# WL-Amigo/waifu2x-converter-cpp

Measured on AMD Instinct MI355X. Metric: Mpixels/sec end-to-end scale2.0x 7-layer conv, higher is better.
Workload: dtype f32; 1 GPU; scale2x_1080p (BASELINE.json configs[1]): scale2.0x topology (1-32-32-64-64-128-128-1, synthetic seeded weights) on a 1920x1080 RGB frame -> Y plane nearest-2x -> 3840x2160 CNN plane, one frame per GPU per step

## Files before the change

### waifu2x-converter-cpp_amd/csrc/w2xc_wino4.hip

```cpp
#include "w2xc_kernels.h"
#include "w2xc_device.h"
#include "w2xc_launch.hpp"
#include "w2xc_layout.h"
#include "w2xc_wino4_math.h"

#include <type_traits>

#ifdef W4_TIMING
__device__ unsigned long long w4_stamps[2][8192];
#define W4_STAMP(idx) do { const int i_ = (idx); if (blockIdx.x == 0 && pt == 0 && lane == 0 && i_ < 8192) w4_stamps[bt][i_] = __builtin_amdgcn_s_memtime(); } while (0)
#else
#define W4_STAMP(idx) do { } while (0)
#endif
#ifndef W4P_T0
#define W4P_T0 3
#endif
#ifndef W4_PF
#define W4_PF 2
#endif
#ifndef W4_DMA4
#define W4_DMA4 1
#endif
#ifndef W4_ABL
#define W4_ABL 0
#endif

namespace {

typedef float f32x4u __attribute__((ext_vector_type(4), aligned(4)));

static constexpr __host__ __device__ int w4p_dd_of(int xi) { return 6 * ((xi % 18) / 3) + 3 * (xi / 18) + (xi % 18) % 3; }

}

static __device__ __forceinline__ void store16_sc1(float *p, f32x4 v) { asm volatile("global_store_dwordx4 %0, %1, off sc1\n\ts_nop 1" : : "v"(p), "v"(v) : "memory"); }
static __device__ __forceinline__ void store4_sc1(float *p, float v) { asm volatile("global_store_dword %0, %1, off sc1\n\ts_nop 1" : : "v"(p), "v"(v) : "memory"); }
static __device__ __forceinline__ void store16_sys(float *p, f32x4 v) { asm volatile("global_store_dwordx4 %0, %1, off sc0 sc1\n\ts_nop 1" : : "v"(p), "v"(v) : "memory"); }
static __device__ __forceinline__ void store4_sys(float *p, float v) { asm volatile("global_store_dword %0, %1, off sc0 sc1\n\ts_nop 1" : : "v"(p), "v"(v) : "memory"); }

template <int K, int N>
static __device__ __forceinline__ void load16_sc1_batch(f32x4 (&t)[N], unsigned voff, const char *const (&b)[N])
{
    if constexpr (K < N) {
        unsigned long long bc;
        asm volatile("s_mov_b64 %1, %3\n\tglobal_load_dwordx4 %0, %2, %1 sc1" : "=v"(t[K]), "=&s"(bc) : "v"(voff), "s"(b[K]) : "memory");
        load16_sc1_batch<K + 1, N>(t, voff, b);
    }
}
template <int K, int N>
static __device__ __forceinline__ void pin_batch(f32x4 (&t)[N])
{
    if constexpr (K < N) {
        asm volatile("" : "+v"(t[K]));
        pin_batch<K + 1, N>(t);
    }
}
template <int K, int N>
static __device__ __forceinline__ void sum_batch(f32x4 &v, const f32x4 (&t)[N])
{
    if constexpr (K < N) {
        v += t[K];
        sum_batch<K + 1, N>(v, t);
    }
}

struct W4ProgJob {
    const float *G; long long ts, gs, rs;
    float *out; long long out_rs;
    const float *bias;
    unsigned *flags; unsigned epoch;
    int g_h, g_w, g_off, wino_py, ngroups;
// ... 38 lines not shown
        pin_batch<0, 9 * NOB>(t1);
        auto finish = [&](bool on, const f32x4 (&t)[9 * NOB], int yy, int xx, bool whole) {
            if (!on) return;
            f32x4 v = {0.0f, 0.0f, 0.0f, 0.0f};
            sum_batch<0, 9 * NOB>(v, t);
            float *oq = outp + (long long)yy * out_rs + xx;
            if (whole) {
                f32x4 o;
#pragma unroll
                for (int e = 0; e < 4; e++) o[e] = leaky(v[e] + b);
                store16_sys(oq, o);
            } else {
                const int sh = xx - (g_w - 4);
                for (int e = 0; xx + e < g_w; e++) {
                    const int idx = sh + e;
                    const float ve = idx == 0 ? v[0] : idx == 1 ? v[1] : idx == 2 ? v[2] : v[3];
                    store4_sys(oq + e, leaky(ve + b));
                }
            }
        };
        finish(true, t0, yy0, xx0, whole0);
        finish(on1, t1, yy1, xx1, whole1);
    }
    unsigned *flags = reinterpret_cast<unsigned *>(uni64((unsigned long long)a.flags));
    if (flags) {
        asm volatile("s_waitcnt vmcnt(0)" ::: "memory");
        __builtin_amdgcn_s_barrier();
        asm volatile("" ::: "memory");
        if (tid == 0) __hip_atomic_store(flags + (jr * uni(a.ngroups) + jg), (unsigned)uni((int)a.epoch), __ATOMIC_RELAXED, __HIP_MEMORY_SCOPE_SYSTEM);
    }
}

template <int CIN, int COUT, bool OUT_PLANAR, bool IN_NHWC = false, bool FUSE7 = false, bool PROG = false>
__global__ void __launch_bounds__(512, 2) conv3x3_wino4(W2xcConvDesc d, int tiles_x, int nitems)
{
#define W4B_ONLY(...)
#define W4B_SEL(b_, s_) s_
#define W4B_OUT d.out
#include "w2xc_wino4_body.inc"
#undef W4B_OUT
#undef W4B_SEL
#undef W4B_ONLY
}

template <int CIN, int COUT, bool FUSE7>
__global__ void __launch_bounds__(512, 2) conv3x3_wino4_batch(W2xcConvDesc d, int tiles_x, int nitems, W2xcBatchDesc bd)
{
    constexpr bool OUT_PLANAR = true, IN_NHWC = false, PROG = false;
#define W4B_ONLY(...) __VA_ARGS__
#define W4B_SEL(b_, s_) b_
#define W4B_OUT (d.out + (long long)(item / bd.items) * bd.out_bs)
#include "w2xc_wino4_body.inc"
#undef W4B_OUT
#undef W4B_SEL
#undef W4B_ONLY
}

template <int CIN, int COUT, bool OUT_PLANAR, bool IN_NHWC>
__global__ void __launch_bounds__(512, 2) conv3x3_wino4_batch_l(W2xcConvDesc d, int tiles_x, int nitems, W2xcBatchDesc bd)
{
    constexpr bool FUSE7 = false, PROG = false;
#define W4B_ONLY(...) __VA_ARGS__
#define W4B_SEL(b_, s_) b_
#define W4B_OUT (d.out + (long long)(item / bd.items) * bd.out_bs)
#include "w2xc_wino4_body.inc"
#undef W4B_OUT
#undef W4B_SEL
#undef W4B_ONLY
}

#ifndef W2XC_WINO4_PART
#define W2XC_WINO4_PART -1
#endif
template <int CIN, int COUT, bool OUT_PLANAR, bool IN_NHWC = false, bool FUSE7 = false, bool PROG = false>
static hipError_t launch_wino4(const W2xcConvDesc &d, hipStream_t stream)
{
    const int tiles_x = (d.out_w + 31) / 32, tiles_y = (d.out_h + (d.wino_py & 3) + 15) / 16;
    const int nitems = tiles_x * tiles_y * (COUT / 64);
    constexpr size_t lds_bytes = 3 * (size_t)(11 * 1024) + 2 * (size_t)(36 * 1024) + 3 * (size_t)(18 * 1024) + COUT * 4 + (PROG ? 16 : 0);
    static_assert(lds_bytes <= 160 * 1024, "LDS budget");
    if constexpr (PROG) {
        if (!d.prog_cnt || !d.g_out || !d.g_bias || d.g_w < 4 || (long long)d.out_h * d.out_rs * 4 >= (1ll << 32)) return hipErrorInvalidValue;
        hipError_t em = hipMemsetAsync(d.prog_cnt, 0, w2xc_wino4_prog_counters(d.out_w, d.out_h, d.wino_py) * sizeof(unsigned), stream);
        if (em != hipSuccess) return em;
    }
    auto kern = conv3x3_wino4<CIN, COUT, OUT_PLANAR, IN_NHWC, FUSE7, PROG>;
    static W2xcLdsOptIn opt_in;
    const hipError_t e = opt_in(kern, lds_bytes);
    if (e != hipSuccess) return e;
    hipLaunchKernelGGL(kern, dim3(w2xc_persistent_grid(nitems)), dim3(512), lds_bytes, stream, d, tiles_x, nitems);
    return hipGetLastError();
}


hipError_t w2xc_launch_wino4_nhwc_out(const W2xcConvDesc &d, hipStream_t stream);
#if W2XC_WINO4_PART == 1 || W2XC_WINO4_PART == -1
hipError_t w2xc_launch_wino4_nhwc_out(const W2xcConvDesc &d, hipStream_t stream)
{
#ifdef W4P_SINGLE
    return hipErrorInvalidValue;
#else
    if (d.cin == 32 && d.in_ps == 32 && d.in_cs == 1)
        return d.cout == 64 ? launch_wino4<32, 64, false, true>(d, stream) : d.cout == 128 ? launch_wino4<32, 128, false, true>(d, stream) : hipErrorInvalidValue;
    switch (d.cin * 1000 + d.cout) {
    case 32064:  return launch_wino4<32, 64, false>(d, stream);
    case 32128:  return launch_wino4<32, 128, false>(d, stream);
    case 64064:  return launch_wino4<64, 64, false>(d, stream);
    case 64128:  return launch_wino4<64, 128, false>(d, stream);
    case 128064: return launch_wino4<128, 64, false>(d, stream);
    case 128128: return launch_wino4<128, 128, false>(d, stream);
    case 128256: return w2xc_launch_wino4_wide(d, stream);
    default: return hipErrorInvalidValue;
    }
#endif
}
#endif

#if W2XC_WINO4_PART == 7 || W2XC_WINO4_PART == -1
hipError_t w2xc_launch_wino4_wide(const W2xcConvDesc &d, hipStream_t stream)
{
    if (d.cin != 128 || d.cout != 256 || d.in_ps != 1 || d.out_ps != 256 || d.out_cs != 1 || d.out_terms == 9) return hipErrorInvalidValue;
    return launch_wino4<128, 256, false>(d, stream);
}
// ... 55 lines not shown
#ifndef W4P_SINGLE
    if (in_nhwc) return d.cout == 64 ? launch_wino4<32, 64, true, true>(d, stream) : d.cout == 128 ? launch_wino4<32, 128, true, true>(d, stream) : hipErrorInvalidValue;
#endif
#ifdef W4P_SINGLE
    return d.cin == 128 && d.cout == 128 ? launch_wino4<128, 128, true>(d, stream) : hipErrorInvalidValue;
#else
    switch (d.cin * 1000 + d.cout) {
    case 32064:  return launch_wino4<32, 64, true>(d, stream);
    case 32128:  return launch_wino4<32, 128, true>(d, stream);
    case 64064:  return launch_wino4<64, 64, true>(d, stream);
    case 64128:  return launch_wino4<64, 128, true>(d, stream);
    case 128064: return launch_wino4<128, 64, true>(d, stream);
    case 128128: return launch_wino4<128, 128, true>(d, stream);
    default: return hipErrorInvalidValue;
    }
#endif
}
#endif

template <int CIN, int COUT, bool FUSE7>
static hipError_t launch_wino4_batch(const W2xcConvDesc &d, W2xcBatchDesc b, hipStream_t stream)
{
    const int tiles_x = (d.out_w + 31) / 32, tiles_y = (d.out_h + (d.wino_py & 3) + 15) / 16;
    const long long items = (long long)tiles_x * tiles_y * (COUT / 64);
    if (items * b.batch >= (1ll << 31)) return hipErrorInvalidValue;
    b.items = (int)items;
    const int nitems = (int)(items * b.batch);
    constexpr size_t lds_bytes = 3 * (size_t)(11 * 1024) + 2 * (size_t)(36 * 1024) + 3 * (size_t)(18 * 1024) + COUT * 4;
    static_assert(lds_bytes <= 160 * 1024, "LDS budget");
    auto kern = conv3x3_wino4_batch<CIN, COUT, FUSE7>;
    static W2xcLdsOptIn opt_in;
    const hipError_t e = opt_in(kern, lds_bytes);
    if (e != hipSuccess) return e;
    hipLaunchKernelGGL(kern, dim3(w2xc_persistent_grid(nitems)), dim3(512), lds_bytes, stream, d, tiles_x, nitems, b);
    return hipGetLastError();
}

template <int CIN, int COUT, bool OUT_PLANAR, bool IN_NHWC>
static hipError_t launch_wino4_batch_l(const W2xcConvDesc &d, W2xcBatchDesc b, hipStream_t stream)
{
    const int tiles_x = (d.out_w + 31) / 32, tiles_y = (d.out_h + (d.wino_py & 3) + 15) / 16;
    const long long items = (long long)tiles_x * tiles_y * (COUT / 64);
    if (items * b.batch >= (1ll << 31)) return hipErrorInvalidValue;
    b.items = (int)items;
    const int nitems = (int)(items * b.batch);
    constexpr size_t lds_bytes = 3 * (size_t)(11 * 1024) + 2 * (size_t)(36 * 1024) + 3 * (size_t)(18 * 1024) + COUT * 4;
    static_assert(lds_bytes <= 160 * 1024, "LDS budget");
    auto kern = conv3x3_wino4_batch_l<CIN, COUT, OUT_PLANAR, IN_NHWC>;
    static W2xcLdsOptIn opt_in;
    const hipError_t e = opt_in(kern, lds_bytes);
    if (e != hipSuccess) return e;
    hipLaunchKernelGGL(kern, dim3(w2xc_persistent_grid(nitems)), dim3(512), lds_bytes, stream, d, tiles_x, nitems, b);
    return hipGetLastError();
}

hipError_t w2xc_launch_wino4_batch_nhwc_in(const W2xcConvDesc &d, W2xcBatchDesc b, hipStream_t stream);
#if W2XC_WINO4_PART == 5 || W2XC_WINO4_PART == -1
hipError_t w2xc_launch_wino4_batch_nhwc_in(const W2xcConvDesc &d, W2xcBatchDesc b, hipStream_t stream)
{
    if (d.out_ps == 1) return d.cout == 64 ? launch_wino4_batch_l<32, 64, true, true>(d, b, stream) : d.cout == 128 ? launch_wino4_batch_l<32, 128, true, true>(d, b, stream) : hipErrorInvalidValue;
    return d.cout == 64 ? launch_wino4_batch_l<32, 64, false, true>(d, b, stream) : d.cout == 128 ? launch_wino4_batch_l<32, 128, false, true>(d, b, stream) : hipErrorInvalidValue;
}
#endif

hipError_t w2xc_launch_wino4_batch_nhwc_out(const W2xcConvDesc &d, W2xcBatchDesc b, hipStream_t stream);
#if W2XC_WINO4_PART == 6 || W2XC_WINO4_PART == -1
hipError_t w2xc_launch_wino4_batch_nhwc_out(const W2xcConvDesc &d, W2xcBatchDesc b, hipStream_t stream)
{
    switch (d.cin * 1000 + d.cout) {
    case 64064:  return launch_wino4_batch_l<64, 64, false, false>(d, b, stream);
    case 64128:  return launch_wino4_batch_l<64, 128, false, false>(d, b, stream);
    case 128064: return launch_wino4_batch_l<128, 64, false, false>(d, b, stream);
    case 128128: return launch_wino4_batch_l<128, 128, false, false>(d, b, stream);
    default: return hipErrorInvalidValue;
    }
}
#endif

hipError_t w2xc_launch_wino4_batch_wide(const W2xcConvDesc &d, W2xcBatchDesc b, hipStream_t stream);
#if W2XC_WINO4_PART == 8 || W2XC_WINO4_PART == -1
hipError_t w2xc_launch_wino4_batch_wide(const W2xcConvDesc &d, W2xcBatchDesc b, hipStream_t stream)
{
    if (d.cin != 128 || d.cout != 256 || d.in_ps != 1 || d.out_ps != 256 || d.out_cs != 1 || d.out_terms == 9) return hipErrorInvalidValue;
    return launch_wino4_batch_l<128, 256, false, false>(d, b, stream);
}
// ... 57 lines not shown
```

### waifu2x-converter-cpp_amd/csrc/w2xc_wino4_body.inc

```
    static_assert(!PROG || FUSE7, "PROG finishes the fused last layer");
    constexpr int ROWS = 16;
    constexpr int NST = CIN / 4;
    constexpr int NOB = COUT / 64;
    constexpr int CHS = 168;
    constexpr int RAW_PIECES = 11;
    constexpr unsigned RAW_BYTES = RAW_PIECES * 1024;
    constexpr unsigned U_BASE = 3 * RAW_BYTES, U_BYTES = 36 * 1024;
    constexpr unsigned V_BASE = U_BASE + 2 * U_BYTES, V_BYTES = 18 * 1024;
    constexpr unsigned SPARE_BASE = V_BASE + 2 * V_BYTES;
    constexpr unsigned BIAS_BASE = SPARE_BASE + V_BYTES;
    static_assert(CIN % 16 == 0 && COUT % 64 == 0 && NST % 4 == 0 && NST >= 8, "planes");
    constexpr int STRIP = 16;
    constexpr int GW = 8;
    constexpr unsigned TRIG_BASE = BIAS_BASE + COUT * 4;
    const int tiles_y = W4B_SEL(bd.items, nitems) / (NOB * tiles_x);
    W4B_ONLY(const int img_tiles = bd.items / NOB;)
    const int pxcd = blockIdx.x & 7;
    auto band_lo = [&](int k, int r) { return (k * tiles_x + (r & 7)) >> 3; };
    auto tile_coords = [&](int pt_, int &ty_, int &tx_) {
        W4B_ONLY(pt_ = pt_ % img_tiles;)
        if constexpr (PROG) {
            const int p8 = pt_ / tiles_x;
            int rem = pt_ - p8 * tiles_x, j = 0, lo = band_lo(pxcd, 0), wd = band_lo(pxcd + 1, 0) - lo;
            while (rem >= wd && j < 7) {
                rem -= wd;
                j++;
                lo = band_lo(pxcd, j);
                wd = band_lo(pxcd + 1, j) - lo;
            }
            ty_ = 8 * p8 + j;
            tx_ = lo + rem;
            return;
        }
        const int per_strip = STRIP * tiles_y;
        int sidx = pt_ / per_strip;
        const int nfull = tiles_x / STRIP;
        if (sidx > nfull) sidx = nfull;
        const int wid = sidx < nfull ? STRIP : tiles_x - nfull * STRIP;
        const int q = pt_ - sidx * per_strip;
        ty_ = q / wid;
        tx_ = sidx * STRIP + (q - ty_ * wid);
    };
    extern __shared__ __attribute__((aligned(16))) float lds[];
    const unsigned lds0 = (unsigned)(size_t)(__attribute__((address_space(3))) float *)lds;
    char *ldsb = reinterpret_cast<char *>(lds);

    const int lane = threadIdx.x & 63;
    const int wave = __builtin_amdgcn_readfirstlane(threadIdx.x >> 6);
    const int pt = wave & 3, bt = wave >> 2;
    const unsigned b_voff = (unsigned)lane * 16u;
    auto lin = [&]() { unsigned v = b_voff; asm volatile("" : "+v"(v)); return v; };
    auto lane_o = [&]() { return (int)(lin() >> 4); };

    const int xcd = blockIdx.x & 7, per = gridDim.x >> 3;
    const int cq = nitems >> 3, cr = nitems & 7;
    int chunk_begin = xcd < cr ? xcd * (cq + 1) : cr * (cq + 1) + (xcd - cr) * cq;
    int chunk_end = chunk_begin + cq + (xcd < cr ? 1 : 0);
    if constexpr (PROG) {
        int nloc = (tiles_y >> 3) * tiles_x;
        for (int j = 0; j < (tiles_y & 7); j++) nloc += band_lo(xcd + 1, j) - band_lo(xcd, j);
        chunk_begin = 0;
        chunk_end = nloc * NOB;
    }
#ifndef W4_PAIR
#define W4_PAIR 0
#endif
    int item0 = chunk_begin + (blockIdx.x >> 3);
    int nmy = (chunk_end - item0 + per - 1) / per;
    if constexpr (W4_PAIR && NOB == 2 && !PROG) {
        const int ntile = nitems >> 1, tq = ntile >> 3, tr = ntile & 7;
        const int tb = xcd < tr ? xcd * (tq + 1) : tr * (tq + 1) + (xcd - tr) * tq, te = tb + tq + (xcd < tr ? 1 : 0);
        item0 = tb + (blockIdx.x >> 3);
        if (item0 >= te) return;
        nmy = 2 * ((te - item0 + per - 1) / per);
    } else if (item0 >= chunk_end) return;
    auto item_of = [&](int n) {
        const int nn = n < nmy ? n : nmy - 1;
        if constexpr (W4_PAIR && NOB == 2 && !PROG) return 2 * (item0 + (nn >> 1) * per) + (nn & 1);
        else return item0 + nn * per;
    };

    for (int c = threadIdx.x; c < COUT; c += 512) lds[BIAS_BASE / 4 + c] = d.bias[c];
    if constexpr (PROG) {
        if (threadIdx.x < 4) lds[TRIG_BASE / 4 + threadIdx.x] = 0.0f;
    }

    const long long cs4 = d.in_cs * 4, rs4 = d.in_rs * 4;
    constexpr int DW = W4_DMA4 ? 4 : 8;
    constexpr int RJ = (RAW_PIECES + DW - 1) / DW;
    constexpr int UQ = 36 / DW + (36 % DW ? 1 : 0);
    unsigned voff[RJ];
    const char *a_base;
    int xlim_r;
    auto tile_offsets = [&](int it) {
        int ty_, tx_;
        tile_coords(it / NOB, ty_, tx_);
        const int lane_t = lane_o();
        const int y0 = ty_ * ROWS - d.wino_py + d.off_y, x0 = tx_ * 32 + d.off_x;
        const int yb = clampi(y0, 0, d.in_h - 1);
        a_base = reinterpret_cast<const char *>(d.in) + (long long)yb * rs4;
        W4B_ONLY(a_base += (long long)(it / bd.items) * bd.in_bs * 4;)
        xlim_r = d.in_w - x0;
        if constexpr (IN_NHWC) {
            xlim_r = 64;
#pragma unroll
            for (int jj = 0; jj < RJ; jj++) {
                int ci = (jj * DW + wave) * 64 + lane_t;
                ci = ci < (ROWS + 2) * 36 ? ci : (ROWS + 2) * 36 - 1;
                const int R = ci / 36, slot = ci - R * 36;
                const int x = 4 * (slot % 9) + slot / 9;
                const int gy = clampi(y0 + R, 0, d.in_h - 1) - yb;
                const int gx = clampi(x0 + x, 0, d.in_w - 1);
                voff[jj] = (unsigned)((long long)gy * rs4 + (long long)gx * (CIN * 4));
            }
            return;
        }
        const int xq_last = (d.in_w - 1) & ~3;
#pragma unroll
        for (int jj = 0; jj < RJ; jj++) {
            const int ci = (jj * DW + wave) * 64 + lane_t;
            int kk = ci / CHS;
            kk = kk < 4 ? kk : 3;
            const int rem = ci - kk * CHS;
            int R = rem / 9;
            const int q = rem - R * 9;
            R = R < ROWS + 2 ? R : ROWS + 1;
            const int gy = clampi(y0 + R, 0, d.in_h - 1) - yb;
            int gx = x0 + 4 * q;
            gx = gx < xq_last ? gx : xq_last;
            voff[jj] = (unsigned)((long long)kk * cs4 + (long long)gy * rs4 + (long long)gx * 4);
        }
    };
    const unsigned wbase = (unsigned)__builtin_amdgcn_readfirstlane(lds0 + (unsigned)wave * 1024u);
    auto dma_raw = [&](auto JJ, unsigned roff, int slice) {
        constexpr int jj = decltype(JJ)::value;
        const char *sbase = a_base + (long long)slice * (IN_NHWC ? 16 : 4 * cs4);
        lds_dma16_si<jj * DW * 1024u>(sbase, voff[jj], wbase + roff);
    };
    const char *wpk_w = reinterpret_cast<const char *>(d.wpk) + (size_t)wave * 1024;
    auto dma_u = [&](int ob, int s_, auto SLOT, auto Q) {
        constexpr unsigned slot = decltype(SLOT)::value;
        constexpr int q = decltype(Q)::value;
        const char *sbase = wpk_w + ((size_t)(ob * NST + s_) * 36 + q * DW) * 1024;
        lds_dma16_si<U_BASE + slot * U_BYTES + q * DW * 1024u>(sbase, b_voff, wbase);
    };
#ifndef W4_DMA_BASES
#define W4_DMA_BASES 1
#endif
    constexpr bool DMAB = W4_DMA_BASES && W4_DMA4 && !(CIN == 32 && COUT == 128 && !OUT_PLANAR && !IN_NHWC && !FUSE7);
    auto dma_u_pair = [&](const char *u_pair, auto SLOT, auto Q) {
// ... 155 lines not shown

    auto run = [&](auto PH_) {
    constexpr int PH = decltype(PH_)::value;
    using C0 = std::integral_constant<int, 0>;
    using C1 = std::integral_constant<int, 1>;
    using U0 = std::integral_constant<unsigned, 0u>;
    lane_regs();
    const unsigned park_u = (bt * 3 + PH - 1) < 4 ? U_BASE + U_BYTES + (unsigned)(bt * 3 + PH - 1) * 9216u : SPARE_BASE + (unsigned)(bt * 3 + PH - 1 - 4) * 9216u;
    auto park = [&]() {
        char *pa = ldsb + (lin() + park_u);
        static_for<0, 9>([&](auto Q_) {
            constexpr int q = decltype(Q_)::value;
            *reinterpret_cast<f32x4 *>(pa + q * 1024) = f32x4{dd[4 * q], dd[4 * q + 1], dd[4 * q + 2], dd[4 * q + 3]};
        });
    };
    auto unpark = [&]() {
        const char *pa = ldsb + (lin() + park_u);
        static_for<0, 9>([&](auto Q_) {
            constexpr int q = decltype(Q_)::value;
            const f32x4 v = *reinterpret_cast<const f32x4 *>(pa + q * 1024);
            dd[4 * q] = v[0]; dd[4 * q + 1] = v[1]; dd[4 * q + 2] = v[2]; dd[4 * q + 3] = v[3];
        });
    };
    auto quarter = [&](auto Q_, const char *src, char *dst, int xlim) {
        constexpr int q = decltype(Q_)::value;
        if constexpr (q == 0) {
            static_for<0, 6>([&](auto I) { raw_read(src, I); });
            raw_mask(xlim);
        }
        if constexpr (q < 2) static_for<3 * q, 3 * q + 3>([&](auto I) { row_pass(I); });
        else static_for<3 * (q - 2), 3 * (q - 2) + 3>([&](auto J) { col_pass(J); });
        if constexpr (q == 3) static_for<0, 9>([&](auto Q) { v_write(dst, Q); });
    };
    tile_offsets(item_of(0));
    int xlim_cur = xlim_r;
    auto raw_all = [&](unsigned roff, int slice) {
        if (wave < DW) {
            static_for<0, RJ - 1>([&](auto JJ) { dma_raw(JJ, roff, slice); });
            if (wave < RAW_PIECES - (RJ - 1) * DW) dma_raw(std::integral_constant<int, RJ - 1>{}, roff, slice);
        }
    };
    for (int sl = 0; sl < 3; sl++) raw_all((unsigned)sl * RAW_BYTES, sl);
    if (wave < DW) {
        const int ob0 = item_of(0) % NOB;
        static_for<0, UQ - 1>([&](auto Q) { dma_u(ob0, 0, U0{}, Q); });
        if (wave < 36 - (UQ - 1) * DW) dma_u(ob0, 0, U0{}, std::integral_constant<int, UQ - 1>{});
    }
    W2XC_WAIT_VMCNT(0);
    __builtin_amdgcn_s_barrier();
    asm volatile("" ::: "memory");
    if constexpr (PH < 3) {
        const char *src = ldsb + PH * RAW_BYTES + tr_rd();
        static_for<0, 4 - PH>([&](auto Q) { quarter(Q, src, ldsb + tr_wr(), xlim_cur); });
    }
    asm volatile("s_waitcnt lgkmcnt(0)" ::: "memory");
    __builtin_amdgcn_s_barrier();
    asm volatile("" ::: "memory");
    for (int sl = 3; sl < 6; sl++) raw_all((unsigned)(sl - 3) * RAW_BYTES, sl);
    W2XC_WAIT_VMCNT(0);
    __builtin_amdgcn_s_barrier();
    asm volatile("" ::: "memory");
    if constexpr (PH == 3) quarter(C0{}, ldsb + tr_rd(), nullptr, xlim_cur);
    asm volatile("s_waitcnt lgkmcnt(0)" ::: "memory");
    __builtin_amdgcn_s_barrier();
    asm volatile("" ::: "memory");

    constexpr int PF = W4_PF;
// ... 4 lines not shown
        const char *va = va_of(slot);
        static_for<0, PF>([&](auto G) {
            constexpr int g = decltype(G)::value;
            const int b = PF == 2 ? g : (int)slot;
            a4[b] = *reinterpret_cast<const f32x4 *>(ua + g * 4096);
            b4[b] = *reinterpret_cast<const f32x4 *>(va + g * 2048);
        });
    };
    unsigned rd = RAW_BYTES, mid = 2 * RAW_BYTES, fr = 0;
    int stamp = 0;
    (void)stamp;
    W4_STAMP(stamp++);
    for (int n = 0; n < nmy; n++) {
        const int item = item_of(n), item_n = item_of(n + 1);
        f32x4 acc[36];

        auto stage = [&](auto J_, auto FIRST_, int s) {
            constexpr int J = decltype(J_)::value;
            constexpr bool FIRST = decltype(FIRST_)::value;
            constexpr int QT = (J - PH) & 3;
            constexpr unsigned par = J & 1, nxt = par ^ 1u;
            int u_ob = item % NOB, u_s = s + 1;
            if (s == NST - 1) { u_ob = item_n % NOB; u_s = 0; }
            const char *ua = ua_of(par);
            const char *va = va_of(par);
            const char *u_st = wpk_w + (size_t)(u_ob * NST + u_s) * 36864, *u_pair = u_st;
            if constexpr (DMAB) asm volatile("" : "+s"(u_st));
            const char *srcQ = nullptr;
            char *dstQ = nullptr;
            if constexpr (QT == 0) srcQ = ldsb + (rd + tr_rd());
            if constexpr (QT == 3) dstQ = ldsb + (tr_wr() + nxt * V_BYTES);
            const int xlimQ = s + 4 < NST ? xlim_cur : xlim_r;
            if constexpr (J == 2) {
                if (s == NST - 6) tile_offsets(item_n);
            }
            const int r_slice = s + 6 < NST ? s + 6 : s + 6 - NST;
            static_for<0, 36>([&](auto XI) {
                constexpr int xi = decltype(XI)::value;
                constexpr int g = xi >> 2;
                if constexpr (xi == 32) {
                    W4_STAMP(stamp++);
                    if constexpr ((W4_ABL & 32) != 0) W2XC_WAIT_VMCNT(0);
                    else if (wave < RAW_PIECES - (RJ - 1) * DW) wait_vmcnt_n(RJ);
                    else if (wave < DW) wait_vmcnt_n(RJ - 1);
                    asm volatile("s_waitcnt lgkmcnt(0)" ::: "memory");
                    W4_STAMP(stamp++);
                    __builtin_amdgcn_s_barrier();
                    asm volatile("" ::: "memory");
                    { const unsigned tr = rd; rd = mid; mid = fr; fr = tr; }
                    if (s != NST - 1) {
                        if constexpr (PF == 2) load_first(nxt);
                        else {
                            a4[nxt] = *reinterpret_cast<const f32x4 *>(ua_of(nxt));
                            b4[nxt] = *reinterpret_cast<const f32x4 *>(va_of(nxt));
                        }
                    }
                    W4_STAMP(stamp++);
                    __builtin_amdgcn_sched_barrier(0);
                }
                if constexpr ((xi & 3) == 0 && g + PF < 9 && !(W4_ABL & 128)) {
                    constexpr int b = PF == 2 ? (g + PF) % 3 : ((g + 1 + (int)par) & 1);
                    a4[b] = *reinterpret_cast<const f32x4 *>(ua + (g + PF) * 4096);
                    b4[b] = *reinterpret_cast<const f32x4 *>(va + (g + PF) * 2048);
                    __builtin_amdgcn_sched_barrier(0);
                }
                {
                    constexpr int b = PF == 2 ? g % 3 : ((g + (int)par) & 1);
// ... 35 lines not shown
                    __builtin_amdgcn_sched_barrier(0);
                }
                if constexpr (QT == 3 && xi >= W4P_T0 + 3 && xi < W4P_T0 + 6) {
                    v_write(dstQ, std::integral_constant<int, 3 * (xi - (W4P_T0 + 3))>{});
                    v_write(dstQ, std::integral_constant<int, 3 * (xi - (W4P_T0 + 3)) + 1>{});
                    v_write(dstQ, std::integral_constant<int, 3 * (xi - (W4P_T0 + 3)) + 2>{});
                    __builtin_amdgcn_sched_barrier(0);
                }
            });
        };
        load_first(0u);
        stage(std::integral_constant<int, 0>{}, std::true_type{}, 0);
#pragma unroll 1
        for (int s = 1; s < NST; s += 4) {
            stage(std::integral_constant<int, 1>{}, std::false_type{}, s);
            stage(std::integral_constant<int, 2>{}, std::false_type{}, s + 1);
            stage(std::integral_constant<int, 3>{}, std::false_type{}, s + 2);
            if (s + 3 < NST) stage(std::integral_constant<int, 0>{}, std::false_type{}, s + 3);
        }
        asm volatile("s_nop 15\n\ts_nop 15" ::: "memory");
        xlim_cur = xlim_r;
        if constexpr (PH != 0) {
            if constexpr (PARK) park();
            else pin_dd();
        }
        {
            __builtin_amdgcn_s_setprio(2);
            const int ob = item % NOB;
            const int lane_e = lane_o(), t = lane_e & 15, k = lane_e >> 4;
            int tile_y, tile_x;
            tile_coords(item / NOB, tile_y, tile_x);
            const int ty0 = tile_y * ROWS - d.wino_py;
            const int oy = ty0 + 4 * (2 * bt + (t >> 3)), ox = tile_x * 32 + 4 * (t & 7);
            const int plane0 = ob * 64 + pt * 16 + 4 * k;
            float *obase = OUT_PLANAR ? W4B_OUT + (long long)plane0 * d.out_cs + (long long)oy * d.out_rs + ox
                                      : W4B_OUT + (long long)oy * d.out_rs + (long long)ox * COUT + plane0;
            const bool interior = ty0 >= 0 && ty0 + ROWS <= d.out_h && tile_x * 32 + 32 <= d.out_w;
            const f32x4 bq = *reinterpret_cast<const f32x4 *>(ldsb + BIAS_BASE + plane0 * 4);
            float a7[4];
            if constexpr (FUSE7) {
                const float *w7 = reinterpret_cast<const float *>(d.w7pk) + (size_t)(ob * 4 + pt) * 256 + lane_e;
#pragma unroll
                for (int e = 0; e < 4; e++) a7[e] = w7[e * 64];
            }
            constexpr bool SLAB_ITEM = FUSE7 && !PARK;
            constexpr int SLAB_PX = SLAB_ITEM ? 512 : 128;
            char *red = ldsb + V_BASE + V_BYTES;
            auto slab_of = [&](int q) {
                if constexpr (SLAB_ITEM) return ldsb + (q < 2 ? U_BASE + U_BYTES + (unsigned)q * V_BYTES : V_BASE + V_BYTES + (unsigned)(q - 2) * V_BYTES);
                else return red + q * (9 * 128 * 4);
            };
            static_assert(SPARE_BASE == V_BASE + 2 * V_BYTES && U_BYTES == 2 * V_BYTES && V_BYTES == 9 * 512 * 4, "the item's slab");
            auto tap_reduce = [&](int job, int tap, int gy, int gx) {
                f32x4 sum = *reinterpret_cast<const f32x4 *>(slab_of(0) + job * 16);
#pragma unroll
                for (int q = 1; q < 4; q++) sum += *reinterpret_cast<const f32x4 *>(slab_of(q) + job * 16);
                if (gy >= 0 && gy < d.out_h && gx < d.out_w) {
                    float *g = W4B_OUT + (long long)ob * d.out_ts + (long long)tap * d.out_gs + (long long)gy * d.out_rs + gx;
                    if constexpr (PROG) {
                        if (gx + 3 < d.out_w) store16_sc1(g, sum);
                        else {
#pragma unroll
                            for (int e = 0; e < 3; e++)
                                if (gx + e < d.out_w) store4_sc1(g + e, sum[e]);
                        }
                    } else if (gx + 3 < d.out_w) *reinterpret_cast<f32x4u *>(g) = sum;
                    else {
#pragma unroll
                        for (int e = 0; e < 3; e++)
                            if (gx + e < d.out_w) g[e] = sum[e];
                    }
                }
            };
            unsigned tick = 0xFFFFFFFFu, pq0 = 0, pq1 = 0;
            (void)tick; (void)pq0; (void)pq1;
            float tm[4][6][4];
#pragma unroll
            for (int e = 0; e < 4; e++)
#pragma unroll
                for (int j = 0; j < 6; j++) {
                    const float m0 = acc[xi_of(0, j)][e], m1 = acc[xi_of(1, j)][e], m2 = acc[xi_of(2, j)][e], m3 = acc[xi_of(3, j)][e],
                                m4 = acc[xi_of(4, j)][e], m5 = acc[xi_of(5, j)][e];
                    const float s1 = m1 + m2, d1 = m1 - m2, s2 = m3 + m4, d2 = m3 - m4;
                    tm[0][j][e] = m0 + s1 + s2;
                    tm[1][j][e] = __builtin_fmaf(1.5f, d2, 0.75f * d1);
                    tm[2][j][e] = __builtin_fmaf(2.25f, s2, 0.5625f * s1);
                    tm[3][j][e] = __builtin_fmaf(3.375f, d2, __builtin_fmaf(0.421875f, d1, m5));
                }
            if constexpr (PROG) W2XC_WAIT_VMCNT(0);
#pragma unroll
            for (int rp = 0; rp < 2; rp++) {
#pragma unroll
                for (int rr = 0; rr < 2; rr++) {
                    const int i = 2 * rp + rr;
                    f32x4 y[4];
#pragma unroll
                    for (int e = 0; e < 4; e++) {
                        float y0, y1, y2, y3;
                        at6(tm[i][0][e], tm[i][1][e], tm[i][2][e], tm[i][3][e], tm[i][4][e], tm[i][5][e], y0, y1, y2, y3);
                        const float w0 = y0 + bq[e], w1 = y1 + bq[e], w2 = y2 + bq[e], w3 = y3 + bq[e];
                        const float l0 = __builtin_amdgcn_fmed3f(w0, 0.1f * w0, 3.402823466e+38f), l1 = __builtin_amdgcn_fmed3f(w1, 0.1f * w1, 3.402823466e+38f);
                        const float l2 = __builtin_amdgcn_fmed3f(w2, 0.1f * w2, 3.402823466e+38f), l3 = __builtin_amdgcn_fmed3f(w3, 0.1f * w3, 3.402823466e+38f);
                        if constexpr (OUT_PLANAR || FUSE7) y[e] = f32x4{l0, l1, l2, l3};
                        else { y[0][e] = l0; y[1][e] = l1; y[2][e] = l2; y[3][e] = l3; }
                    }
// ... 3 lines not shown
                        for (int j = 0; j < 4; j++) D[j] = f32x4{0.0f, 0.0f, 0.0f, 0.0f};
#pragma unroll
                        for (int e = 0; e < 4; e++)
#pragma unroll
                            for (int j = 0; j < 4; j++) D[j] = __builtin_amdgcn_mfma_f32_16x16x4f32(a7[e], y[e][j], D[j], 0, 0, 0);
                        const int p0 = (SLAB_ITEM ? i * 128 : 0) + (2 * bt + (t >> 3)) * 32 + (t & 7) * 4;
                        char *slab = slab_of(pt);
                        if (k < 2) {
#pragma unroll
                            for (int r = 0; r < 4; r++) *reinterpret_cast<f32x4 *>(slab + ((4 * k + r) * SLAB_PX + p0) * 4) = f32x4{D[0][r], D[1][r], D[2][r], D[3][r]};
                        } else if (k == 2) {
                            *reinterpret_cast<f32x4 *>(slab + (8 * SLAB_PX + p0) * 4) = f32x4{D[0][0], D[1][0], D[2][0], D[3][0]};
                        }
                        if constexpr (!SLAB_ITEM) {
                            asm volatile("s_waitcnt lgkmcnt(0)" ::: "memory");
                            __builtin_amdgcn_s_barrier();
                            asm volatile("" ::: "memory");
                            if constexpr (PROG) {
                                if (i == 0 && wave == CW) prog_early(n > 0 ? item_of(n - 1) : -1, tick, pq0, pq1);
                                if (i == 3 && wave == CW) prog_late(n > 0 ? item_of(n - 1) : -1, tick, pq0, pq1);
                            }
                            {
                                const int tid = wave * 64 + lane_e;
                                if (tid < 288) {
                                    const int tap = tid >> 5, p = (tid & 31) * 4;
                                    tap_reduce(tid, tap, ty0 + 4 * (p >> 5) + i, tile_x * 32 + (p & 31));
                                }
                            }
                            asm volatile("s_waitcnt lgkmcnt(0)" ::: "memory");
                            __builtin_amdgcn_s_barrier();
                            asm volatile("" ::: "memory");
                        }
                    } else if constexpr ((W4_ABL & 64) != 0) {
                        if (y[0][0] == 12345.678f) *reinterpret_cast<f32x4 *>(obase) = y[0] + y[1] + y[2] + y[3];
                    } else if constexpr (OUT_PLANAR) {
                        if (interior || (oy + i >= 0 && oy + i < d.out_h && ox < d.out_w)) {
#pragma unroll
                            for (int e = 0; e < 4; e++) *reinterpret_cast<f32x4 *>(obase + (long long)e * d.out_cs + (long long)i * d.out_rs) = y[e];
                        }
                    } else if (interior) {
#pragma unroll
                        for (int j = 0; j < 4; j++) *reinterpret_cast<f32x4 *>(obase + (long long)i * d.out_rs + j * COUT) = y[j];
                    } else {
#pragma unroll
                        for (int j = 0; j < 4; j++)
                            if (oy + i >= 0 && oy + i < d.out_h && ox + j < d.out_w) *reinterpret_cast<f32x4 *>(obase + (long long)i * d.out_rs + j * COUT) = y[j];
                    }
                }
            }
            if constexpr (SLAB_ITEM) {
                asm volatile("s_waitcnt lgkmcnt(0)" ::: "memory");
                __builtin_amdgcn_s_barrier();
                asm volatile("" ::: "memory");
                const int tid = wave * 64 + lane_e;
#pragma unroll
                for (int jb = 0; jb < 3; jb++) {
                    const int job = tid + jb * 512;
                    if (jb < 2 || job < 9 * 128) {
                        const int tap = job >> 7, i = (job >> 5) & 3, p = (job & 31) * 4;
                        tap_reduce(job, tap, ty0 + 4 * (p >> 5) + i, tile_x * 32 + (p & 31));
                    }
                }
                asm volatile("s_waitcnt lgkmcnt(0)" ::: "memory");
                __builtin_amdgcn_s_barrier();
                asm volatile("" ::: "memory");
            }
            __builtin_amdgcn_s_setprio(0);
            W4_STAMP(stamp++);
            if constexpr (PROG) prog_run();
        }
        if constexpr (PARK) {
            if constexpr (PH != 0) unpark();
            asm volatile("s_waitcnt lgkmcnt(0)" ::: "memory");
            __builtin_amdgcn_s_barrier();
            asm volatile("" ::: "memory");
        } else {
            if constexpr (PH != 0) pin_dd();
            lane_regs();
        }
    }
    W2XC_WAIT_VMCNT(0);
    if constexpr (PROG) {
        __builtin_amdgcn_s_barrier();
        asm volatile("" ::: "memory");
        bool first = true;
        for (;;) {
            if (wave == CW) {
                unsigned tick, q0, q1;
                prog_early(first ? item_of(nmy - 1) : -1, tick, q0, q1);
                prog_late(first ? item_of(nmy - 1) : -1, tick, q0, q1);
                unsigned t = *lds_ticket;
                if (*lds_action == 0 && t) {
                    unsigned q = 0;
                    while ((q = __hip_atomic_load(q_slots + (t - 1), __ATOMIC_RELAXED, __HIP_MEMORY_SCOPE_AGENT)) == 0) __builtin_amdgcn_s_sleep(8);
// ... 26 lines not shown
```

Before: 148.7 Mpix/s (input-image pixels; CNN-plane pixels = 4x).

## Precompute tile geometry reciprocals and use SGPR-base plus 32-bit offset stores

Adds a host-computed geometry struct holding reciprocals, so tile and image index divisions in the kernel become multiply-high operations. Output stores switch to a scalar base plus 32-bit per-lane offset form when the offsets fit, which cuts 64-bit vector address arithmetic. Input tile offsets are cached for interior tiles so the per-lane offsets are not recomputed. This adds code complexity and needs an extra kernel argument, and it relies on the range checks to keep the reciprocal division and 32-bit offsets correct.

```diff
diff --git a/waifu2x-converter-cpp_amd/csrc/w2xc_wino4.hip b/waifu2x-converter-cpp_amd/csrc/w2xc_wino4.hip
--- a/waifu2x-converter-cpp_amd/csrc/w2xc_wino4.hip
+++ b/waifu2x-converter-cpp_amd/csrc/w2xc_wino4.hip
@@ -3,6 +3,7 @@
 #include "w2xc_launch.hpp"
 #include "w2xc_layout.h"
 #include "w2xc_wino4_math.h"
+#include "w2xc_wino4_geom.h"
 
 #include <type_traits>
 
@@ -37,6 +38,14 @@
 static __device__ __forceinline__ void store4_sc1(float *p, float v) { asm volatile("global_store_dword %0, %1, off sc1\n\ts_nop 1" : : "v"(p), "v"(v) : "memory"); }
 static __device__ __forceinline__ void store16_sys(float *p, f32x4 v) { asm volatile("global_store_dwordx4 %0, %1, off sc0 sc1\n\ts_nop 1" : : "v"(p), "v"(v) : "memory"); }
 static __device__ __forceinline__ void store4_sys(float *p, float v) { asm volatile("global_store_dword %0, %1, off sc0 sc1\n\ts_nop 1" : : "v"(p), "v"(v) : "memory"); }
+
+template <int IMM = 0>
+static __device__ __forceinline__ void store16_sv(const void *sbase, unsigned voff, f32x4 v)
+{
+    static_assert(IMM >= 0 && IMM <= 4095, "global_store immediate offset");
+    unsigned long long b;
+    asm volatile("s_mov_b64 %0, %3\n\tglobal_store_dwordx4 %1, %2, %0 offset:%4\n\ts_nop 1" : "=&s"(b) : "v"(voff), "v"(v), "s"(sbase), "n"(IMM) : "memory");
+}
 
 template <int K, int N>
 static __device__ __forceinline__ void load16_sc1_batch(f32x4 (&t)[N], unsigned voff, const char *const (&b)[N])
@@ -141,7 +150,7 @@
 }
 
 template <int CIN, int COUT, bool OUT_PLANAR, bool IN_NHWC = false, bool FUSE7 = false, bool PROG = false>
-__global__ void __launch_bounds__(512, 2) conv3x3_wino4(W2xcConvDesc d, int tiles_x, int nitems)
+__global__ void __launch_bounds__(512, 2) conv3x3_wino4(W2xcConvDesc d, int tiles_x, int nitems, W4Geom geo)
 {
 #define W4B_ONLY(...)
 #define W4B_SEL(b_, s_) s_
@@ -153,12 +162,12 @@
 }
 
 template <int CIN, int COUT, bool FUSE7>
-__global__ void __launch_bounds__(512, 2) conv3x3_wino4_batch(W2xcConvDesc d, int tiles_x, int nitems, W2xcBatchDesc bd)
+__global__ void __launch_bounds__(512, 2) conv3x3_wino4_batch(W2xcConvDesc d, int tiles_x, int nitems, W2xcBatchDesc bd, W4Geom geo)
 {
     constexpr bool OUT_PLANAR = true, IN_NHWC = false, PROG = false;
 #define W4B_ONLY(...) __VA_ARGS__
 #define W4B_SEL(b_, s_) b_
-#define W4B_OUT (d.out + (long long)(item / bd.items) * bd.out_bs)
+#define W4B_OUT (d.out + (long long)img_of(item) * bd.out_bs)
 #include "w2xc_wino4_body.inc"
 #undef W4B_OUT
 #undef W4B_SEL
@@ -166,12 +175,12 @@
 }
 
 template <int CIN, int COUT, bool OUT_PLANAR, bool IN_NHWC>
-__global__ void __launch_bounds__(512, 2) conv3x3_wino4_batch_l(W2xcConvDesc d, int tiles_x, int nitems, W2xcBatchDesc bd)
+__global__ void __launch_bounds__(512, 2) conv3x3_wino4_batch_l(W2xcConvDesc d, int tiles_x, int nitems, W2xcBatchDesc bd, W4Geom geo)
 {
     constexpr bool FUSE7 = false, PROG = false;
 #define W4B_ONLY(...) __VA_ARGS__
 #define W4B_SEL(b_, s_) b_
-#define W4B_OUT (d.out + (long long)(item / bd.items) * bd.out_bs)
+#define W4B_OUT (d.out + (long long)img_of(item) * bd.out_bs)
 #include "w2xc_wino4_body.inc"
 #undef W4B_OUT
 #undef W4B_SEL
@@ -197,7 +206,8 @@
     static W2xcLdsOptIn opt_in;
     const hipError_t e = opt_in(kern, lds_bytes);
     if (e != hipSuccess) return e;
-    hipLaunchKernelGGL(kern, dim3(w2xc_persistent_grid(nitems)), dim3(512), lds_bytes, stream, d, tiles_x, nitems);
+    const W4Geom geo = w4_geom(tiles_x, tiles_y, COUT / 64, w4_lane32(FUSE7 ? 0 : d.out_cs, d.out_rs, COUT));
+    hipLaunchKernelGGL(kern, dim3(w2xc_persistent_grid(nitems)), dim3(512), lds_bytes, stream, d, tiles_x, nitems, geo);
     return hipGetLastError();
 }
 
@@ -319,7 +329,8 @@
     static W2xcLdsOptIn opt_in;
     const hipError_t e = opt_in(kern, lds_bytes);
     if (e != hipSuccess) return e;
-    hipLaunchKernelGGL(kern, dim3(w2xc_persistent_grid(nitems)), dim3(512), lds_bytes, stream, d, tiles_x, nitems, b);
+    const W4Geom geo = w4_geom(tiles_x, tiles_y, COUT / 64, w4_lane32(FUSE7 ? 0 : d.out_cs, d.out_rs, COUT));
+    hipLaunchKernelGGL(kern, dim3(w2xc_persistent_grid(nitems)), dim3(512), lds_bytes, stream, d, tiles_x, nitems, b, geo);
     return hipGetLastError();
 }
 
@@ -337,7 +348,8 @@
     static W2xcLdsOptIn opt_in;
     const hipError_t e = opt_in(kern, lds_bytes);
     if (e != hipSuccess) return e;
-    hipLaunchKernelGGL(kern, dim3(w2xc_persistent_grid(nitems)), dim3(512), lds_bytes, stream, d, tiles_x, nitems, b);
+    const W4Geom geo = w4_geom(tiles_x, tiles_y, COUT / 64, w4_lane32(d.out_cs, d.out_rs, COUT));
+    hipLaunchKernelGGL(kern, dim3(w2xc_persistent_grid(nitems)), dim3(512), lds_bytes, stream, d, tiles_x, nitems, b, geo);
     return hipGetLastError();
 }
 
diff --git a/waifu2x-converter-cpp_amd/csrc/w2xc_wino4_body.inc b/waifu2x-converter-cpp_amd/csrc/w2xc_wino4_body.inc
--- a/waifu2x-converter-cpp_amd/csrc/w2xc_wino4_body.inc
+++ b/waifu2x-converter-cpp_amd/csrc/w2xc_wino4_body.inc
@@ -10,17 +10,17 @@
     constexpr unsigned SPARE_BASE = V_BASE + 2 * V_BYTES;
     constexpr unsigned BIAS_BASE = SPARE_BASE + V_BYTES;
     static_assert(CIN % 16 == 0 && COUT % 64 == 0 && NST % 4 == 0 && NST >= 8, "planes");
-    constexpr int STRIP = 16;
     constexpr int GW = 8;
     constexpr unsigned TRIG_BASE = BIAS_BASE + COUT * 4;
-    const int tiles_y = W4B_SEL(bd.items, nitems) / (NOB * tiles_x);
-    W4B_ONLY(const int img_tiles = bd.items / NOB;)
+    const int tiles_y = geo.tiles_y;
+    auto img_of = [&](int it_) { return (int)w4_div((unsigned)it_, geo.img_items, geo.r_img_items); };
+    (void)img_of;
     const int pxcd = blockIdx.x & 7;
     auto band_lo = [&](int k, int r) { return (k * tiles_x + (r & 7)) >> 3; };
     auto tile_coords = [&](int pt_, int &ty_, int &tx_) {
-        W4B_ONLY(pt_ = pt_ % img_tiles;)
+        W4B_ONLY(pt_ -= (int)(w4_div((unsigned)pt_, geo.img_tiles, geo.r_img_tiles) * geo.img_tiles);)
         if constexpr (PROG) {
-            const int p8 = pt_ / tiles_x;
+            const int p8 = (int)w4_div((unsigned)pt_, (unsigned)tiles_x, geo.r_tiles_x);
             int rem = pt_ - p8 * tiles_x, j = 0, lo = band_lo(pxcd, 0), wd = band_lo(pxcd + 1, 0) - lo;
             while (rem >= wd && j < 7) {
                 rem -= wd;
@@ -32,14 +32,7 @@
             tx_ = lo + rem;
             return;
         }
-        const int per_strip = STRIP * tiles_y;
-        int sidx = pt_ / per_strip;
-        const int nfull = tiles_x / STRIP;
-        if (sidx > nfull) sidx = nfull;
-        const int wid = sidx < nfull ? STRIP : tiles_x - nfull * STRIP;
-        const int q = pt_ - sidx * per_strip;
-        ty_ = q / wid;
-        tx_ = sidx * STRIP + (q - ty_ * wid);
+        w4_tile_of(geo, pt_, ty_, tx_);
     };
     extern __shared__ __attribute__((aligned(16))) float lds[];
     const unsigned lds0 = (unsigned)(size_t)(__attribute__((address_space(3))) float *)lds;
@@ -92,17 +85,50 @@
     unsigned voff[RJ];
     const char *a_base;
     int xlim_r;
-    auto tile_offsets = [&](int it) {
+    int voff_inner = 0;
+    auto tile_offsets = [&](int it, auto FAST_) {
+        constexpr bool FAST = decltype(FAST_)::value;
         int ty_, tx_;
         tile_coords(it / NOB, ty_, tx_);
+        const int y0 = ty_ * ROWS - d.wino_py + d.off_y, x0 = tx_ * 32 + d.off_x;
+        xlim_r = IN_NHWC ? 64 : d.in_w - x0;
+        if (!PROG && wave >= DW) return;
+        const char *in_b = reinterpret_cast<const char *>(d.in);
+        W4B_ONLY(in_b += (long long)img_of(it) * bd.in_bs * 4;)
+        const int xq_last = (d.in_w - 1) & ~3;
+        constexpr int PX = IN_NHWC ? CIN * 4 : 4;
+        const bool inner = FAST && !PROG && y0 >= 0 && y0 + ROWS + 1 <= d.in_h - 1 && (IN_NHWC ? x0 >= 0 && x0 + 35 <= d.in_w - 1 : x0 + 32 <= xq_last);
+        if (inner) {
+            a_base = in_b + (long long)y0 * rs4 + (long long)x0 * PX;
+            if (!voff_inner) {
+                voff_inner = 1;
+                const int lane_t = lane_o();
+#pragma unroll
+                for (int jj = 0; jj < RJ; jj++) {
+                    int ci = (jj * DW + wave) * 64 + lane_t;
+                    if constexpr (IN_NHWC) {
+                        ci = ci < (ROWS + 2) * 36 ? ci : (ROWS + 2) * 36 - 1;
+                        const int R = ci / 36, slot = ci - R * 36;
+                        const int x = 4 * (slot % 9) + slot / 9;
+                        voff[jj] = (unsigned)((long long)R * rs4 + (long long)x * PX);
+                    } else {
+                        int kk = ci / CHS;
+                        kk = kk < 4 ? kk : 3;
+                        const int rem = ci - kk * CHS;
+                        int R = rem / 9;
+                        const int q = rem - R * 9;
+                        R = R < ROWS + 2 ? R : ROWS + 1;
+                        voff[jj] = (unsigned)((long long)kk * cs4 + (long long)R * rs4 + (long long)q * 16);
+                    }
+                }
+            }
+            return;
+        }
+        voff_inner = 0;
         const int lane_t = lane_o();
-        const int y0 = ty_ * ROWS - d.wino_py + d.off_y, x0 = tx_ * 32 + d.off_x;
         const int yb = clampi(y0, 0, d.in_h - 1);
-        a_base = reinterpret_cast<const char *>(d.in) + (long long)yb * rs4;
-        W4B_ONLY(a_base += (long long)(it / bd.items) * bd.in_bs * 4;)
-        xlim_r = d.in_w - x0;
+        a_base = in_b + (long long)yb * rs4;
         if constexpr (IN_NHWC) {
-            xlim_r = 64;
 #pragma unroll
             for (int jj = 0; jj < RJ; jj++) {
                 int ci = (jj * DW + wave) * 64 + lane_t;
@@ -115,7 +141,6 @@
             }
             return;
         }
-        const int xq_last = (d.in_w - 1) & ~3;
 #pragma unroll
         for (int jj = 0; jj < RJ; jj++) {
             const int ci = (jj * DW + wave) * 64 + lane_t;
@@ -337,7 +362,7 @@
         else static_for<3 * (q - 2), 3 * (q - 2) + 3>([&](auto J) { col_pass(J); });
         if constexpr (q == 3) static_for<0, 9>([&](auto Q) { v_write(dst, Q); });
     };
-    tile_offsets(item_of(0));
+    tile_offsets(item_of(0), std::false_type{});
     int xlim_cur = xlim_r;
     auto raw_all = [&](unsigned roff, int slice) {
         if (wave < DW) {
@@ -408,7 +433,7 @@
             if constexpr (QT == 3) dstQ = ldsb + (tr_wr() + nxt * V_BYTES);
             const int xlimQ = s + 4 < NST ? xlim_cur : xlim_r;
             if constexpr (J == 2) {
-                if (s == NST - 6) tile_offsets(item_n);
+                if (s == NST - 6) tile_offsets(item_n, std::true_type{});
             }
             const int r_slice = s + 6 < NST ? s + 6 : s + 6 - NST;
             static_for<0, 36>([&](auto XI) {
@@ -510,9 +535,18 @@
             tile_coords(item / NOB, tile_y, tile_x);
             const int ty0 = tile_y * ROWS - d.wino_py;
             const int oy = ty0 + 4 * (2 * bt + (t >> 3)), ox = tile_x * 32 + 4 * (t & 7);
-            const int plane0 = ob * 64 + pt * 16 + 4 * k;
-            float *obase = OUT_PLANAR ? W4B_OUT + (long long)plane0 * d.out_cs + (long long)oy * d.out_rs + ox
-                                      : W4B_OUT + (long long)oy * d.out_rs + (long long)ox * COUT + plane0;
+            const int plane_w = ob * 64 + pt * 16, plane0 = plane_w + 4 * k;
+            float *const sbase = OUT_PLANAR ? W4B_OUT + (long long)plane_w * d.out_cs + (long long)(ty0 + 8 * bt) * d.out_rs + tile_x * 32
+                                            : W4B_OUT + (long long)(ty0 + 8 * bt) * d.out_rs + (long long)(tile_x * 32) * COUT + plane_w;
+            unsigned long long la;
+            if (geo.lane32)
+                la = OUT_PLANAR ? (unsigned)k * (unsigned)(d.out_cs * 16) + (unsigned)(t >> 3) * (unsigned)(d.out_rs * 16) + (unsigned)(t & 7) * 16u
+                                : (unsigned)(t >> 3) * (unsigned)(d.out_rs * 16) + (unsigned)(t & 7) * (unsigned)(COUT * 16) + (unsigned)k * 16u;
+            else
+                la = (unsigned long long)(OUT_PLANAR ? W4B_OUT + (long long)plane0 * d.out_cs + (long long)oy * d.out_rs + ox
+                                                     : W4B_OUT + (long long)oy * d.out_rs + (long long)ox * COUT + plane0);
+            float *row_p = sbase;
+            (void)row_p;
             const bool interior = ty0 >= 0 && ty0 + ROWS <= d.out_h && tile_x * 32 + 32 <= d.out_w;
             const f32x4 bq = *reinterpret_cast<const f32x4 *>(ldsb + BIAS_BASE + plane0 * 4);
             float a7[4];
@@ -529,26 +563,31 @@
                 else return red + q * (9 * 128 * 4);
             };
             static_assert(SPARE_BASE == V_BASE + 2 * V_BYTES && U_BYTES == 2 * V_BYTES && V_BYTES == 9 * 512 * 4, "the item's slab");
+            auto tap_sum = [&](int job) {
+                f32x4 sum = *reinterpret_cast<const f32x4 *>(slab_of(0) + job * 16);
+#pragma unroll
+                for (int q = 1; q < 4; q++) sum += *reinterpret_cast<const f32x4 *>(slab_of(q) + job * 16);
+                return sum;
+            };
+            auto tap_put = [&](float *tp, f32x4 sum, int gx, bool whole) {
+                if constexpr (PROG) {
+                    if (whole) store16_sc1(tp, sum);
+                    else {
+#pragma unroll
+                        for (int e = 0; e < 3; e++)
+                            if (gx + e < d.out_w) store4_sc1(tp + e, sum[e]);
+                    }
+                } else if (whole) *reinterpret_cast<f32x4u *>(tp) = sum;
+                else {
+#pragma unroll
+                    for (int e = 0; e < 3; e++)
+                        if (gx + e < d.out_w) tp[e] = sum[e];
+                }
+            };
+            auto tap_at = [&](int tap, int gy, int gx) { return W4B_OUT + (long long)ob * d.out_ts + (long long)tap * d.out_gs + (long long)gy * d.out_rs + gx; };
             auto tap_reduce = [&](int job, int tap, int gy, int gx) {
-                f32x4 sum = *reinterpret_cast<const f32x4 *>(slab_of(0) + job * 16);
-#pragma unroll
-                for (int q = 1; q < 4; q++) sum += *reinterpret_cast<const f32x4 *>(slab_of(q) + job * 16);
-                if (gy >= 0 && gy < d.out_h && gx < d.out_w) {
-                    float *g = W4B_OUT + (long long)ob * d.out_ts + (long long)tap * d.out_gs + (long long)gy * d.out_rs + gx;
-                    if constexpr (PROG) {
-                        if (gx + 3 < d.out_w) store16_sc1(g, sum);
-                        else {
-#pragma unroll
-                            for (int e = 0; e < 3; e++)
-                                if (gx + e < d.out_w) store4_sc1(g + e, sum[e]);
-                        }
-                    } else if (gx + 3 < d.out_w) *reinterpret_cast<f32x4u *>(g) = sum;
-                    else {
-#pragma unroll
-                        for (int e = 0; e < 3; e++)
-                            if (gx + e < d.out_w) g[e] = sum[e];
-                    }
-                }
+                const f32x4 sum = tap_sum(job);
+                if (gy >= 0 && gy < d.out_h && gx < d.out_w) tap_put(tap_at(tap, gy, gx), sum, gx, gx + 3 < d.out_w);
             };
             unsigned tick = 0xFFFFFFFFu, pq0 = 0, pq1 = 0;
             (void)tick; (void)pq0; (void)pq1;
@@ -618,19 +657,37 @@
                             asm volatile("" ::: "memory");
                         }
                     } else if constexpr ((W4_ABL & 64) != 0) {
-                        if (y[0][0] == 12345.678f) *reinterpret_cast<f32x4 *>(obase) = y[0] + y[1] + y[2] + y[3];
+                        if (y[0][0] == 12345.678f) *reinterpret_cast<f32x4 *>(la) = y[0] + y[1] + y[2] + y[3];
                     } else if constexpr (OUT_PLANAR) {
-                        if (interior || (oy + i >= 0 && oy + i < d.out_h && ox < d.out_w)) {
-#pragma unroll
-                            for (int e = 0; e < 4; e++) *reinterpret_cast<f32x4 *>(obase + (long long)e * d.out_cs + (long long)i * d.out_rs) = y[e];
+                        if (interior || ((unsigned)(oy + i) < (unsigned)d.out_h && ox < d.out_w)) {
+                            if (geo.lane32) {
+                                float *sb = row_p;
+#pragma unroll
+                                for (int e = 0; e < 4; e++) {
+                                    store16_sv(sb, (unsigned)la, y[e]);
+                                    if (e < 3) { sb += d.out_cs; asm volatile("" : "+s"(sb)); }
+                                }
+                            } else {
+                                float *const obase = reinterpret_cast<float *>(la);
+#pragma unroll
+                                for (int e = 0; e < 4; e++) *reinterpret_cast<f32x4 *>(obase + (long long)e * d.out_cs + (long long)i * d.out_rs) = y[e];
+                            }
                         }
-                    } else if (interior) {
-#pragma unroll
-                        for (int j = 0; j < 4; j++) *reinterpret_cast<f32x4 *>(obase + (long long)i * d.out_rs + j * COUT) = y[j];
+                    } else if (geo.lane32) {
+                        float *const sb_i = row_p;
+                        const bool row_in = interior || (unsigned)(oy + i) < (unsigned)d.out_h;
+                        static_for<0, 4>([&](auto J) {
+                            constexpr int j = decltype(J)::value;
+                            if (interior || (row_in && ox + j < d.out_w)) store16_sv<j * COUT * 4>(sb_i, (unsigned)la, y[j]);
+                        });
                     } else {
+                        float *const obase = reinterpret_cast<float *>(la);
 #pragma unroll
                         for (int j = 0; j < 4; j++)
-                            if (oy + i >= 0 && oy + i < d.out_h && ox + j < d.out_w) *reinterpret_cast<f32x4 *>(obase + (long long)i * d.out_rs + j * COUT) = y[j];
+                            if (interior || ((unsigned)(oy + i) < (unsigned)d.out_h && ox + j < d.out_w)) *reinterpret_cast<f32x4 *>(obase + (long long)i * d.out_rs + j * COUT) = y[j];
+                    }
+                    if constexpr (!FUSE7) {
+                        if (i < 3) { row_p += d.out_rs; asm volatile("" : "+s"(row_p)); }
                     }
                 }
             }
@@ -639,13 +696,20 @@
                 __builtin_amdgcn_s_barrier();
                 asm volatile("" ::: "memory");
                 const int tid = wave * 64 + lane_e;
+                const int gy_l = (lane_e >> 5) + 4 * ((lane_e & 31) >> 3), gy = ty0 + 2 * (wave & 1) + gy_l, gx = tile_x * 32 + 4 * (lane_e & 7);
+                const bool ok = interior || ((unsigned)gy < (unsigned)d.out_h && gx < d.out_w), whole = interior || gx + 3 < d.out_w;
+                float *sb_t = W4B_OUT + (long long)ob * d.out_ts + (long long)(wave >> 1) * d.out_gs + (long long)(ty0 + 2 * (wave & 1)) * d.out_rs + tile_x * 32;
+                const unsigned lo_t = (unsigned)gy_l * (unsigned)(d.out_rs * 4) + (unsigned)(lane_e & 7) * 16u;
 #pragma unroll
                 for (int jb = 0; jb < 3; jb++) {
-                    const int job = tid + jb * 512;
-                    if (jb < 2 || job < 9 * 128) {
-                        const int tap = job >> 7, i = (job >> 5) & 3, p = (job & 31) * 4;
-                        tap_reduce(job, tap, ty0 + 4 * (p >> 5) + i, tile_x * 32 + (p & 31));
+                    if (jb < 2 || wave < 2) {
+                        const f32x4 sum = tap_sum(tid + jb * 512);
+                        if (ok) {
+                            if (geo.lane32 && whole) store16_sv(sb_t, lo_t, sum);
+                            else tap_put(tap_at((wave >> 1) + 4 * jb, gy, gx), sum, gx, whole);
+                        }
                     }
+                    if (jb < 2) { sb_t += 4 * d.out_gs; asm volatile("" : "+s"(sb_t)); }
                 }
                 asm volatile("s_waitcnt lgkmcnt(0)" ::: "memory");
                 __builtin_amdgcn_s_barrier();
diff --git a/waifu2x-converter-cpp_amd/csrc/w2xc_wino4_geom.h b/waifu2x-converter-cpp_amd/csrc/w2xc_wino4_geom.h
--- /dev/null
+++ b/waifu2x-converter-cpp_amd/csrc/w2xc_wino4_geom.h
@@ -0,0 +1,59 @@
+#pragma once
+
+#if defined(__HIP__)
+#define W4G_HD __host__ __device__
+#else
+#define W4G_HD
+#endif
+
+W4G_HD inline unsigned w4_recip(unsigned d) { return d <= 1 ? (d ? 0xFFFFFFFFu : 0u) : (unsigned)(0x100000000ull / d); }
+W4G_HD inline unsigned w4_div(unsigned n, unsigned d, unsigned r)
+{
+    unsigned q = (unsigned)(((unsigned long long)n * r) >> 32);
+    if (n - q * d >= d) q++;
+    return q;
+}
+
+struct W4Geom {
+    int tiles_x, tiles_y;
+    int nfull;
+    int wid_last;
+    unsigned per_strip;
+    unsigned r_per_strip, r_wid_last;
+    unsigned r_tiles_x;
+    unsigned img_tiles, r_img_tiles, img_items, r_img_items;
+    int lane32;
+};
+
+W4G_HD inline bool w4_lane32(long long out_cs, long long out_rs, int cout)
+{
+    if (out_cs < 0 || out_rs < 0 || out_cs >= (1ll << 40) || out_rs >= (1ll << 40)) return false;
+    return 4 * (12 * out_cs + 16 * out_rs + 28ll * cout) + 112 < (1ll << 32);
+}
+
+W4G_HD inline W4Geom w4_geom(int tiles_x, int tiles_y, int nob, bool lane32)
+{
+    W4Geom w;
+    w.tiles_x = tiles_x; w.tiles_y = tiles_y;
+    w.nfull = tiles_x / 16;
+    w.wid_last = tiles_x - w.nfull * 16;
+    w.per_strip = 16u * (unsigned)tiles_y;
+    w.r_per_strip = w4_recip(w.per_strip);
+    w.r_wid_last = w4_recip((unsigned)w.wid_last);
+    w.r_tiles_x = w4_recip((unsigned)tiles_x);
+    w.img_tiles = (unsigned)tiles_x * (unsigned)tiles_y;
+    w.r_img_tiles = w4_recip(w.img_tiles);
+    w.img_items = w.img_tiles * (unsigned)nob;
+    w.r_img_items = w4_recip(w.img_items);
+    w.lane32 = lane32 ? 1 : 0;
+    return w;
+}
+
+W4G_HD inline void w4_tile_of(const W4Geom &w, int pt, int &ty, int &tx)
+{
+    int sidx = (int)w4_div((unsigned)pt, w.per_strip, w.r_per_strip);
+    if (sidx > w.nfull) sidx = w.nfull;
+    const int q = pt - sidx * (int)w.per_strip;
+    ty = sidx < w.nfull ? q >> 4 : (int)w4_div((unsigned)q, (unsigned)w.wid_last, w.r_wid_last);
+    tx = sidx * 16 + (q - ty * (sidx < w.nfull ? 16 : w.wid_last));
+}
```

Measured after the change: 149.9 Mpix/s (input-image pixels; CNN-plane pixels = 4x), median of 6. About the same (+0.8%).
